# facebook/facebook360_dep

Hardware: AMD Instinct MI355X
Metric: depth Mpix/s per GPU (full pyramid, 16-cam 2048^2 rig); % HBM-read roofline (higher is better)
Workload: dtype f32+f64; 1 GPU; BASELINE config 3: 16-camera 2048x2048 synthetic rig, 8-frame sequence, full 10-level pyramid per frame, per-level temporal filter (+-2 frames); the same sequence for every --gpus N (block partition, 8 frame(s) on this rank); rig=cfg2, cameras=16, frames=8, temporal_filter=True, halo_transport=local, parallelism=frames x1

## Files before the change

### facebook360_dep_amd/csrc/derp_capi.hip

```cpp
#include <hip/hip_runtime.h>

#include <algorithm>
#include <cfloat>
#include <cmath>
#include <cstdarg>
#include <cstdio>
#include <cstdlib>
#include <cstring>
#include <map>
#include <memory>
#include <string>
#include <vector>

#include <rocprim/device/device_radix_sort.hpp>

#include "../../include/derp_hip.h"
#include "derp_host.h"
#include "derp_kernels.h"
#include "derp_mesh.h"
#include "derp_points.h"
#include "derp_render.h"
#include "derp_geometric.h"
#include "derp_sweep.h"

// ... 135 lines not shown
    coeffs[i] *= sum;
  }
}

int get_lanczos(derp_ctx* c, int ssize, int dsize, LanczosTab** out) {
  auto key = std::make_pair(ssize, dsize);
  auto it = c->lanczos.find(key);
  if (it != c->lanczos.end()) {
    *out = &it->second;
    return 0;
  }
  std::vector<int> ofs(dsize);
  std::vector<float> coef((size_t)dsize * 8);
  const double scale = (double)ssize / dsize;
  for (int d = 0; d < dsize; ++d) {
    float f = (float)((d + 0.5) * scale - 0.5);
    int s = (int)f;
    s -= (s > f);
    f -= s;
    ofs[d] = s;
    lanczos_coeffs(f, &coef[(size_t)d * 8]);
  }
  LanczosTab t;
  ALLOC(c, t.ofs, ofs.size() * sizeof(int));
  ALLOC(c, t.coef, coef.size() * sizeof(float));
  HIPCHK(c, hipMemcpyAsync(t.ofs.p, ofs.data(), ofs.size() * sizeof(int), hipMemcpyHostToDevice, c->stream));
  HIPCHK(c, hipMemcpyAsync(t.coef.p, coef.data(), coef.size() * sizeof(float), hipMemcpyHostToDevice, c->stream));
  HIPCHK(c, hipStreamSynchronize(c->stream));
  *out = &(c->lanczos[key] = std::move(t));
  return 0;
}

int get_area_tab(derp_ctx* c, int ssize, int dsize, AreaTabDev** out, bool forceTable = false) {
  auto key = std::make_pair(forceTable ? -ssize : ssize, dsize);
  auto it = c->areaTabs.find(key);
  if (it != c->areaTabs.end()) {
    *out = &it->second;
    return 0;
  }
  AreaTabDev t;
  const double scale = (double)ssize / dsize;
  const int iscale = (int)std::nearbyint(scale);
  std::vector<int> start(dsize + 1, 0), si;
  std::vector<float> alpha;
  if (!forceTable && iscale >= 1 && std::abs(scale - iscale) < 2.220446049250313e-16) {
    t.iscale = iscale;
// ... 96 lines not shown
  return locs;
}

int ensure_spiral(derp_ctx* c, int radius) {
  if (c->spiralRadius == radius) {
    return 0;
  }
  const std::vector<int2> s = make_spiral(radius * 2 + 1);
  ALLOC(c, c->spiral, s.size() * sizeof(int2));
  HIPCHK(c, hipMemcpy(c->spiral.p, s.data(), s.size() * sizeof(int2), hipMemcpyHostToDevice));
  c->spiralN = (int)s.size();
  c->spiralRadius = radius;
  return 0;
}

int upsample_lanczos_dev(derp_ctx* c, const float* in, int sw, int sh, float* out, int dw, int dh, int planes,
                         size_t inStride, size_t outStride) {
  if (sw == dw && sh == dh) {
    return fail(c, "upsample to identical size not supported");
  }
  LanczosTab *tx, *ty;
  TRY(get_lanczos(c, sw, dw, &tx));
  TRY(get_lanczos(c, sh, dh, &ty));
  const size_t tmpStride = (size_t)dw * sh;
  ALLOC(c, c->w.lanczosTmp, tmpStride * planes * sizeof(float));
  hipLaunchKernelGGL(k_lanczos_h, grid2d(dw, sh, planes, kBlk2d), kBlk2d, 0, c->stream, in, sw, sh, dw,
                     tx->ofs.as<int>(), tx->coef.as<float>(), c->w.lanczosTmp.as<float>(), inStride, tmpStride);
  KCHECK(c);
  hipLaunchKernelGGL(k_lanczos_v, grid2d(dw, dh, planes, kBlk2d), kBlk2d, 0, c->stream, c->w.lanczosTmp.as<float>(), sh,
                     dw, dh, ty->ofs.as<int>(), ty->coef.as<float>(), out, tmpStride, outStride);
  KCHECK(c);
  return 0;
}

int upsample_masked_dev(derp_ctx* c, const float* in, const uint8_t* mask, int sw, int sh, const uint8_t* maskUp,
                        const float* bgUp, float* out, int dw, int dh, int planes = 1) {
  const float scale = float(dw) / float(sw);
  const int radius = (int)(scale * scale + 1);
  TRY(ensure_spiral(c, radius));
  ALLOC(c, c->w.lanczosTmp, (size_t)dw * dh * planes * sizeof(float));
  hipLaunchKernelGGL(k_upsample_nearest_masked, grid2d(dw, dh, planes, kBlk2d), kBlk2d, 0, c->stream, in, mask, sw, sh,
                     maskUp, dw, dh, c->w.lanczosTmp.as<float>());
  KCHECK(c);
  hipLaunchKernelGGL(k_spiral_fill, grid2d(dw, dh, planes, kBlk2d), kBlk2d, 0, c->stream, c->w.lanczosTmp.as<float>(), bgUp,
                     maskUp, dw, dh, c->spiral.as<int2>(), c->spiralN, out);
  KCHECK(c);
// ... 136 lines not shown
  const int tiles = tilesX * tilesY;
  const size_t lds = kCostLdsPerSrc * (size_t)(c->S);
  const int run = std::min(std::max(c->bruteRun, 1), kNumDepths);
  hipLaunchKernelGGL(k_brute_costs, dim3(tiles, (kNumDepths + run - 1) / run, nd), dim3(kCostBlock), lds, c->stream, V,
                     c->w.bruteCost.as<float>(), c->w.bruteConf.as<float>(), tilesX, tiles, run);
  KCHECK(c);
  hipLaunchKernelGGL(k_brute_select, grid2d(V.W, V.H, nd, kBlk2d), kBlk2d, 0, c->stream, V, c->w.bruteCost.as<float>(),
                     c->w.bruteConf.as<float>());
  KCHECK(c);
  hipLaunchKernelGGL(k_brute_margin, grid2d(V.W, V.H, nd, kBlk2d), kBlk2d, 0, c->stream, V);
  KCHECK(c);
  return 0;
}

int run_random_proposals(derp_ctx* c, int dst0, int nd) {
  const int L = c->cur;
  if (c->opt.random_proposals <= 0 || L == c->numLevels - 1) {
    return 0;
  }
  Span sp(c, ST_RANDOM, L);
  c->randomRanThisLevel = true;
  LevelView V = make_view(c, ST_RANDOM, dst0, nd);
  if (V.H > 2 && V.W > 2) {
    hipLaunchKernelGGL(k_row_rank, dim3(V.H - 2, nd), dim3(256), 0, c->stream, V, c->w.rank.as<int>());
    KCHECK(c);
  }
  int tilesX;
  const int tiles = tiles_of(V.W, V.H, tilesX);
  const size_t lds = lds_for_waves(kCostLdsPerSrc * (size_t)(c->S), c->randomWaves, c->ldsPerCu, kCostLdsStatic);
  const CostGrid cg = cost_grid(c, tiles, tilesX, true);
  TRY(block_trace_attach(c, V, 0, cg.blocks, nd));
  const bool four = cost_four_waves(c);
  const auto kernel = cg.perBlock > 1 ? (four ? k_random_proposals_walk : k_random_proposals_walk_w3)
                                      : (four ? k_random_proposals : k_random_proposals_w3);
  hipLaunchKernelGGL(kernel, dim3(cg.blocks, nd), dim3(kCostBlock), lds, c->stream, V, c->w.rank.as<int>(), tilesX, cg.bands, cg.perBlock);
  KCHECK(c);
  return 0;
}

int run_ping_pong(derp_ctx* c, int dst0, int nd) {
  const int L = c->cur;
  if (L == c->numLevels - 1) {
    return 0;
  }
  Span sp(c, ST_PINGPONG, L);
  LevelView V = make_view(c, ST_PINGPONG, dst0, nd);
  const size_t n = (size_t)V.W * V.H;
// ... 135 lines not shown
  if (level < 0 || level >= c->numLevels) {
    return fail(c, "level %d out of range [0, %d)", level, c->numLevels);
  }
  if (c->LW[level] <= 0 || c->LH[level] <= 0) {
    return fail(c, "level %d was declared absent in derp_set_pyramid", level);
  }
  return 0;
}

int level_begin(derp_ctx* c, int level, bool buildAllTables) {
  TRY(check_level(c, level));
  if (c->S - 1 > kMaxSrc) {
    return fail(c, "too many source cameras (%d > %d)", c->S, kMaxSrc + 1);
  }
  c->cur = level;
  const int W = c->LW[level], H = c->LH[level];
  const size_t n = (size_t)W * H;
  if (W < 3 || H < 3) {
    return fail(c, "level %d is too small (%dx%d)", level, W, H);
  }
  TRY(compute_fov_and_masks(c, level));
  {
    Span sp(c, ST_VARIANCE, level);
    hipLaunchKernelGGL(k_variance, grid2d(W, H, c->S, kBlk2d), kBlk2d, 0, c->stream, c->frame().color[level].as<ushort4>(),
                       W, H, c->w.srcVar.as<float>());
    KCHECK(c);
  }
  {
    Span sp(c, ST_OWN_BIAS, level);
    hipLaunchKernelGGL(k_blur3_u16, blur_grid(W, H, c->S), kBlurBlk, 0, c->stream,
                       c->frame().color[level].as<ushort4>(), 0, c->w.ownBias.as<ushort4>(), 0, W, H, n, n);
    KCHECK(c);
  }
  HIPCHK(c, hipMemsetAsync(c->w.cost.p, 0, n * c->D * sizeof(float), c->stream));
  HIPCHK(c, hipMemsetAsync(c->w.confidence.p, 0, n * c->D * sizeof(float), c->stream));
  c->w.mismatchMaskHeld = level <= c->opt.mismatches_start_level && level != c->numLevels - 1;
  if (c->w.mismatchMaskHeld) {
    HIPCHK(c, hipMemsetAsync(c->w.mismatchMask.p, 0, n * c->D, c->stream));
  }
  if (level < c->numLevels - 1 && !c->frame().haveDisp[level + 1] && !buildAllTables) {
    return fail(c, "Missing disparity of level %d needed to start level %d", level + 1, level);
  }
  if (level < c->numLevels - 1 && c->frame().haveDisp[level + 1]) {
    Span sp(c, ST_UPSAMPLE, level);
    const int sw = c->LW[level + 1], sh = c->LH[level + 1];
    if (!c->opt.use_foreground_masks) {
      TRY(upsample_lanczos_dev(c, c->frame().disp[level + 1].as<float>(), sw, sh, c->w.disparity.as<float>(), W, H, c->D,
                               (size_t)sw * sh, n));
    } else {
      ALLOC(c, c->w.staging, (size_t)sw * sh * c->D);
      hipLaunchKernelGGL(k_fov_mask, grid2d(sw, sh, c->D, kBlk2d), kBlk2d, 0, c->stream, c->camsDst.as<Cam>(), sw, sh,
                         c->w.staging.as<uint8_t>());
      KCHECK(c);
      hipLaunchKernelGGL(k_and_masks, dim3(flat_grid((size_t)sw * sh), c->D), dim3(256), 0, c->stream,
// ... 791 lines not shown
```

### facebook360_dep_amd/csrc/derp_ctx.h

```cpp
#pragma once

namespace {

enum Stage {
  ST_FOV = 0,
  ST_VARIANCE,
  ST_OWN_BIAS,
  ST_UPSAMPLE,
  ST_PROJ_WARP,
  ST_REPROJECT,
  ST_PROJ_BIAS,
  ST_BRUTE,
  ST_RANDOM,
  ST_PINGPONG,
  ST_MISMATCH,
  ST_BILATERAL,
  ST_MEDIAN,
  ST_MASKFOV,
  ST_TEMPORAL,
  ST_LANES,
  ST_GC_PREPARE,
  ST_GC_SWEEP,
  ST_GC_CLEAN,
  ST_SWEEP_OVERLAPS,
  ST_SWEEP_EQUIRECT,
  ST_COUNT
};
const char* kStageNames[ST_COUNT] = {"fov_mask",  "variance",    "own_bias",         "upsample",  "proj_warp",
                                     "reproject", "proj_bias",   "brute_force",      "random_proposals",
                                     "ping_pong", "mismatches",  "bilateral",        "median",    "mask_fov",
                                     "temporal",  "lanes_wall", "gc_prepare",       "gc_sweep",  "gc_clean",
                                     "sweep_overlaps", "sweep_equirect"};
constexpr int kMaxLevels = 24;

struct TimedSpan {
  int stage, level;
  hipEvent_t a, b;
};

struct LanczosTab {
  DevBuf ofs, coef;
};

struct AreaTabDev {
  DevBuf start, si, alpha;
  int iscale = 0;
};

struct WorkSet {
  DevBuf srcVar, ownBias, maskAnd, disparity, cost, confidence, dispRes, costRes, changed, tmpF, rank, mismatchMask, pairCount;
  DevBuf tileSeen;
  DevBuf projColor, projBias;
  DevBuf projColorT;
  DevBuf bruteCost, bruteConf, lanczosTmp, staging, stagingB;
  bool mismatchMaskHeld = false;
  int colorTablesCleanLevel = -1;
};

struct FramePyramid {
  std::vector<DevBuf> color, fg, bg, disp;
  std::vector<char> haveBg, haveDisp;
};

struct WorkLane {
  hipStream_t stream = nullptr;
  hipEvent_t done = nullptr;
  WorkSet w;
};

struct SmrState; struct RephotoState; struct PointsState; struct MeshState; struct GcState; struct SweepState;

}

// ... 99 lines not shown
```

### facebook360_dep_amd/csrc/derp_debug_api.h

```cpp
#pragma once

namespace {
struct HostPairs {
  SsdPair* p;
  SsdPair get(int i) const {
    return p[i];
  }
  void set(int i, const SsdPair& v) {
    p[i] = v;
  }
};
int stage_index(const char* stage) {
  for (int i = 0; i < ST_COUNT; ++i) {
    if (strcmp(stage, kStageNames[i]) == 0) {
      return i;
    }
  }
  return -1;
}
}

int derp_debug_atan2_ypos(derp_ctx* c, const double* y, const double* x, double* out, size_t n) {
  if (!c || !y || !x || !out) {
    return fail(c, "bad arguments");
// ... 53 lines not shown
  }
  ALLOC(c, c->w.staging, 9 * n * sizeof(double));
  double* d = c->w.staging.as<double>();
  HIPCHK(c, hipMemcpyAsync(d, xyz, 3 * n * sizeof(double), hipMemcpyHostToDevice, c->stream));
  hipLaunchKernelGGL(k_debug_sees, dim3(flat_grid(n)), dim3(256), 0, c->stream, c->camsSrc.as<Cam>(), src, d, d + 3 * n, n);
  KCHECK(c);
  HIPCHK(c, hipMemcpyAsync(out, d + 3 * n, 6 * n * sizeof(double), hipMemcpyDeviceToHost, c->stream));
  HIPCHK(c, hipStreamSynchronize(c->stream));
  return 0;
}

int derp_debug_download(derp_ctx* c, int d, int s, int which, void* out) {
  TRY(need_current(c, false));
  const int L = c->cur;
  const int W = c->LW[L], H = c->LH[L];
  const size_t n = (size_t)W * H;
  HIPCHK(c, hipStreamSynchronize(c->stream));
  if (which == 4) {
    HIPCHK(c, hipMemcpy(out, c->w.srcVar.as<float>() + (size_t)s * n, n * sizeof(float), hipMemcpyDeviceToHost));
    return 0;
  }
  if (which == 5) {
    HIPCHK(c, hipMemcpy(out, c->fovMask.as<uint8_t>() + (size_t)d * n, n, hipMemcpyDeviceToHost));
    return 0;
  }
  if (d < 0 || d >= c->D || s < 0 || s >= c->S || s == c->dst2srcH[d]) {
    return fail(c, "bad (dst, src) pair");
  }
  const size_t tab = (size_t)d * (c->S - 1) + (s < c->dst2srcH[d] ? s : s - 1);
  if (which == 0) {
    const int PW = W + 2 * kPadW, PH = H + 2 * kPadW;
    std::vector<float2> tmp((size_t)PW * PH);
    HIPCHK(c, hipMemcpy(tmp.data(), c->projWarp.as<float2>() + tab * tmp.size(), tmp.size() * sizeof(float2),
                        hipMemcpyDeviceToHost));
    float2* o = reinterpret_cast<float2*>(out);
    for (int y = 0; y < H; ++y) {
      memcpy(o + (size_t)y * W, &tmp[(size_t)(y + kPadW) * PW + kPadW], (size_t)W * sizeof(float2));
    }
    return 0;
  }
  if (which == 2 || which == 3) {
    const int PW = W + 2 * kPadC, PH = H + 2 * kPadC;
    std::vector<ushort4> tmp((size_t)PW * PH);
    const ushort4* base = (which == 2 ? c->w.projColor.as<ushort4>() : c->w.projBias.as<ushort4>()) + tab * tmp.size();
    HIPCHK(c, hipMemcpy(tmp.data(), base, tmp.size() * sizeof(ushort4), hipMemcpyDeviceToHost));
    uint16_t* o = reinterpret_cast<uint16_t*>(out);
// ... 251 lines not shown
```

### facebook360_dep_amd/csrc/derp_kernels.h

```cpp
#pragma once
#include <hip/hip_runtime.h>
#include <math.h>
#include <stdint.h>

#include <type_traits>

#include "derp_camera.h"
#include "gcc_algos.h"

namespace derp {

#ifndef DERP_COST_MIN_WAVES
#define DERP_COST_MIN_WAVES 4
#endif
#ifndef DERP_RANDOM_MIN_WAVES
#define DERP_RANDOM_MIN_WAVES 4
#endif
#ifndef DERP_RANDOM_TILED
#define DERP_RANDOM_TILED 0
#endif
#ifndef DERP_MIX_HOT_ONLY
#define DERP_MIX_HOT_ONLY 0
#endif
#ifndef DERP_PHASE_TIMERS
// ... 853 lines not shown

__global__ void k_fov_mask(const Cam* __restrict__ cams, int W, int H, uint8_t* __restrict__ out) {
  const int d = blockIdx.z;
  const int x = blockIdx.x * blockDim.x + threadIdx.x, y = blockIdx.y * blockDim.y + threadIdx.y;
  if (x >= W || y >= H) {
    return;
  }
  const Cam& c = cams[d];
  const double px = (x + 0.5) / (double)W, py = (y + 0.5) / (double)H;
  out[(size_t)d * W * H + (size_t)y * W + x] =
      !outside_image_circle(c, px, py, c.principal[0], c.principal[1], c.focal[0], c.focal[1]);
}

__device__ __forceinline__ int reflect101(int p, int len) {
  if (len == 1) {
    return 0;
  }
  while (p < 0 || p >= len) {
    p = p < 0 ? -p : 2 * len - 2 - p;
  }
  return p;
}

__global__ void k_variance(const ushort4* __restrict__ color, int W, int H, float* __restrict__ var) {
  const int s = blockIdx.z;
  const int x = blockIdx.x * blockDim.x + threadIdx.x, y = blockIdx.y * blockDim.y + threadIdx.y;
  if (x >= W || y >= H) {
    return;
  }
  const ushort4* img = color + (size_t)s * W * H;
  const float scale = 1.0f / 65535.0f;
  double sum[3] = {0, 0, 0}, sumSq[3] = {0, 0, 0};
  const int xs[3] = {reflect101(x - 1, W), x, reflect101(x + 1, W)};
  for (int j = -1; j <= 1; ++j) {
    const int yy = reflect101(y + j, H);
    double rs[3], rq[3];
    {
      const ushort4 q0 = img[(size_t)yy * W + xs[0]], q1 = img[(size_t)yy * W + xs[1]], q2 = img[(size_t)yy * W + xs[2]];
      const float f0[3] = {q0.x * scale, q0.y * scale, q0.z * scale};
      const float f1[3] = {q1.x * scale, q1.y * scale, q1.z * scale};
      const float f2[3] = {q2.x * scale, q2.y * scale, q2.z * scale};
      for (int c = 0; c < 3; ++c) {
        rs[c] = (double)f0[c] + (double)f1[c] + (double)f2[c];
        rq[c] = (double)(f0[c] * f0[c]) + (double)(f1[c] * f1[c]) + (double)(f2[c] * f2[c]);
      }
    }
    for (int c = 0; c < 3; ++c) {
      sum[c] += rs[c];
      sumSq[c] += rq[c];
    }
  }
  const double k = 1. / 9;
  float v[3];
  for (int c = 0; c < 3; ++c) {
    const float mean = (float)(sum[c] * k);
    const float meanSq = (float)(sumSq[c] * k);
    v[c] = meanSq - mean * mean;
  }
  const float t = v[0] * 0.3333f + v[1] * 0.3334f;
  var[(size_t)s * W * H + (size_t)y * W + x] = t * 1.0f + v[2] * 0.3333f;
}

constexpr int kBlurRows = 8;
__device__ __forceinline__ ushort4 blur3_texel(const ushort4* __restrict__ img, int IW, int padIn, int W, int H, int x,
                                               int y) {
  unsigned s0 = 0, s1 = 0, s2 = 0;
  for (int j = -1; j <= 1; ++j) {
    const int yy = reflect101(y + j, H) + padIn;
    for (int i = -1; i <= 1; ++i) {
      const int xx = reflect101(x + i, W) + padIn;
      const ushort4 q = img[(size_t)yy * IW + xx];
      s0 += q.x;
      s1 += q.y;
      s2 += q.z;
    }
  }
  return make_ushort4((unsigned short)((s0 + 4) / 9), (unsigned short)((s1 + 4) / 9), (unsigned short)((s2 + 4) / 9), 0);
}
__global__ void k_blur3_u16(const ushort4* __restrict__ in, int padIn, ushort4* __restrict__ out, int padOut, int W,
                            int H, size_t planeIn, size_t planeOut) {
  const int p = blockIdx.z;
  const int ox = blockIdx.x * blockDim.x + threadIdx.x;
  const int oy0 = (blockIdx.y * blockDim.y + threadIdx.y) * kBlurRows;
  const int OW = W + 2 * padOut, OH = H + 2 * padOut;
  if (ox >= OW || oy0 >= OH) {
    return;
  }
  const ushort4* img = in + (size_t)p * planeIn;
  ushort4* dst = out + (size_t)p * planeOut;
  const int IW = W + 2 * padIn;
  const int x = ox - padOut, y0 = oy0 - padOut;
  if (x >= 1 && x <= W - 2 && y0 >= 1 && y0 + kBlurRows - 1 <= H - 2) {
    auto hsum = [&](int y, unsigned (&h)[3]) {
      const ushort4* r = img + (size_t)(y + padIn) * IW + (x + padIn);
      const ushort4 a = r[-1], b = r[0], c = r[1];
      h[0] = (unsigned)a.x + b.x + c.x;
      h[1] = (unsigned)a.y + b.y + c.y;
      h[2] = (unsigned)a.z + b.z + c.z;
    };
    unsigned hp[3], hc[3], hn[3];
    hsum(y0 - 1, hp);
    hsum(y0, hc);
#pragma unroll
    for (int r = 0; r < kBlurRows; ++r) {
      hsum(y0 + r + 1, hn);
      dst[(size_t)(oy0 + r) * OW + ox] =
          make_ushort4((unsigned short)((hp[0] + hc[0] + hn[0] + 4) / 9), (unsigned short)((hp[1] + hc[1] + hn[1] + 4) / 9),
                       (unsigned short)((hp[2] + hc[2] + hn[2] + 4) / 9), 0);
#pragma unroll
      for (int c = 0; c < 3; ++c) {
        hp[c] = hc[c];
        hc[c] = hn[c];
      }
    }
    return;
  }
  const int xc = min(max(x, 0), W - 1);
  for (int r = 0; r < kBlurRows && oy0 + r < OH; ++r) {
    const int yc = min(max(y0 + r, 0), H - 1);
    dst[(size_t)(oy0 + r) * OW + ox] = blur3_texel(img, IW, padIn, W, H, xc, yc);
  }
}

__global__ void k_proj_warp(LevelView V, float2* __restrict__ projWarp) {
  const int s = blockIdx.z;
  const int ox = blockIdx.x * blockDim.x + threadIdx.x, oy = blockIdx.y * blockDim.y + threadIdx.y;
  const int OW = V.W + 2 * kPadW, OH = V.H + 2 * kPadW;
  if (ox >= OW || oy >= OH) {
    return;
  }
  const int x = min(max(ox - kPadW, 0), V.W - 1), y = min(max(oy - kPadW, 0), V.H - 1);
  const Cam& cs = V.camsSrc[s];
  const double W = V.W, H = V.H;
  const double sprx = cs.principal[0] * W, spry = cs.principal[1] * H, sfx = cs.focal[0] * W, sfy = cs.focal[1] * H;
  const double px = x + 0.5, py = y + 0.5;
  const bool outside = outside_image_circle(cs, px, py, sprx, spry, sfx, sfy);
  D3 rig = {0, 0, 0};
  if (!outside) {
    const D3 dir = rig_direction(cs, px, py, sprx, spry, sfx, sfy);
    rig = {cs.pos[0] + dir.x * 1e4, cs.pos[1] + dir.y * 1e4, cs.pos[2] + dir.z * 1e4};
  }
  const size_t plane = (size_t)OW * OH;
  const float nan = __builtin_nanf("");
// ... 518 lines not shown
  const int own = V.dst2src[d];
  const size_t n = (size_t)V.W * V.H, idx = (size_t)y * V.W + x;
  if (!V.srcFg[(size_t)own * n + idx]) {
    V.disparity[(size_t)d * n + idx] = V.bgDisp[(size_t)d * n + idx];
    return;
  }
  const int yy = min(max(y, 1), V.H - 2), xx = min(max(x, 1), V.W - 2);
  const size_t src = (size_t)yy * V.W + xx;
  V.disparity[(size_t)d * n + idx] = V.disparity[(size_t)d * n + src];
  V.cost[(size_t)d * n + idx] = V.cost[(size_t)d * n + src];
  V.confidence[(size_t)d * n + idx] = V.confidence[(size_t)d * n + src];
}

__device__ __forceinline__ bool random_gate(const LevelView& V, int d, int own, size_t idx) {
  const size_t n = (size_t)V.W * V.H;
  if (!V.fovMask[(size_t)d * n + idx] || !V.srcFg[(size_t)own * n + idx]) {
    return false;
  }
  const float varHighDev = 0.1f * V.varHighThresh;
  const float thresh = fmaxf(varHighDev, V.varNoiseFloor);
  return !(V.srcVar[(size_t)own * n + idx] < thresh);
}

__global__ void __launch_bounds__(256) k_row_rank(LevelView V, int* __restrict__ rank) {
  __shared__ int partial[256];
  const int d = V.dst0 + blockIdx.y, y = blockIdx.x + 1;
  const int own = V.dst2src[d];
  const size_t n = (size_t)V.W * V.H;
  const int inner = V.W - 2;
  const int per = (inner + 255) / 256;
  const int x0 = 1 + threadIdx.x * per, x1 = min(x0 + per, V.W - 1);
  int cnt = 0;
  for (int x = x0; x < x1; ++x) {
    cnt += random_gate(V, d, own, (size_t)y * V.W + x);
  }
  partial[threadIdx.x] = cnt;
  __syncthreads();
  for (int off = 1; off < 256; off <<= 1) {
    const int v = ((int)threadIdx.x >= off) ? partial[threadIdx.x - off] : 0;
    __syncthreads();
    partial[threadIdx.x] += v;
    __syncthreads();
  }
  const int run = partial[threadIdx.x] - cnt;
  uint32_t state = minstd_jump(minstd_seed(y * V.level), (uint64_t)V.randomProposals * (uint64_t)run);
  const uint32_t aP = minstd_jump(1u, (uint64_t)V.randomProposals);
  for (int x = x0; x < x1; ++x) {
    rank[(size_t)d * n + (size_t)y * V.W + x] = (int)state;
    if (random_gate(V, d, own, (size_t)y * V.W + x)) {
      state = minstd_mulmod(state, aP);
    }
  }
}

__device__ __forceinline__ void random_proposals_tile(const LevelView& V, const int* __restrict__ rank, int dl, int x, int y, bool go,
                                                      const PatchWin* win, LdsPairs& pairs) {
  const int d = V.dst0 + dl;
  const int own = V.dst2src[d];
  const size_t n = (size_t)V.W * V.H;
  const unsigned idx = (unsigned)y * (unsigned)V.W + (unsigned)x;
  float* disp = V.disparity + (size_t)d * n;
  unsigned nCost = 0, nPair = 0, nSlots = 0, nSlotsFirst = 0;
  PhaseTimers tm;
  const unsigned tk0 = phase_clock();
  if (go) {
    PixCtx px;
    load_pixctx<false>(V, d, own, x, y, win, px);
    const unsigned cull = behind_sources(V, d, idx);
    float currDisp = at32(disp, idx);
    float currCost = 0.f, costThresh = 0.f, amplitude = 0.f;
    const int spare = V.S - 1;
    const float maxDisp = 1.0f / V.minDepthM;
    uint32_t state = (uint32_t)at32(rank + (size_t)d * n, idx);
// ... 712 lines not shown
  if (mask[idx]) {
    const float4 centre = bilateral_texel<GUIDE_U16>(guideV, idx, result);
    const float denom = 2.0f * (sigma * sigma);
    const double rcpDenom = 1.0 / (double)denom;
    float sumWeight = 0.f, weightedAvg = 0.f;
    for (int v = -radius; v <= radius; ++v) {
      const size_t row = (size_t)min(max(y + v, 0), H - 1) * W;
      for (int u = -radius; u <= radius; ++u) {
        const size_t j = row + min(max(x + u, 0), W - 1);
        if (!mask[j]) {
          continue;
        }
        bilateral_tap(centre, bilateral_texel<GUIDE_U16>(guideV, j, image[j]), weight0, weight1, weight2, rcpDenom,
                      expTab, sumWeight, weightedAvg);
      }
    }
    if (sumWeight != 0.0f) {
      result = weightedAvg / sumWeight;
    }
  }
  out[idx] = result;
}

__device__ __forceinline__ void cswap(float& a, float& b) {
  const float lo = fminf(a, b), hi = fmaxf(a, b);
  a = lo;
  b = hi;
}

__global__ void k_masked_median(const float* __restrict__ image, const float* __restrict__ background,
                                const uint8_t* __restrict__ mask, int W, int H, int radius, float* __restrict__ out,
                                size_t planeStride, const uint8_t* __restrict__ fovForNan) {
  const int p = blockIdx.z;
  const int x = blockIdx.x * blockDim.x + threadIdx.x, y = blockIdx.y * blockDim.y + threadIdx.y;
  if (x >= W || y >= H) {
    return;
  }
  const size_t idx = (size_t)y * W + x;
  const float* img = image + (size_t)p * planeStride;
  const uint8_t* m = mask + (size_t)p * planeStride;
  float result = 0.0f;
  if (!m[idx]) {
    if (background) {
      result = background[(size_t)p * planeStride + idx];
    }
  } else if (radius == 1) {
    const float inf = __builtin_inff();
    float v[9];
    int cnt = 0;
#pragma unroll
    for (int j = 0; j < 3; ++j) {
#pragma unroll
      for (int i = 0; i < 3; ++i) {
        const int yy = y + j - 1, xx = x + i - 1;
        float t = inf;
        if (yy >= 0 && yy < H && xx >= 0 && xx < W) {
          const size_t q = (size_t)yy * W + xx;
          const float val = img[q];
          if (m[q] && !isnan(val) && val != 0) {
            t = val;
            ++cnt;
          }
        }
        v[j * 3 + i] = t;
      }
    }
    cswap(v[0], v[1]); cswap(v[3], v[4]); cswap(v[6], v[7]);
    cswap(v[1], v[2]); cswap(v[4], v[5]); cswap(v[7], v[8]);
    cswap(v[0], v[1]); cswap(v[3], v[4]); cswap(v[6], v[7]);
    cswap(v[0], v[3]); cswap(v[3], v[6]); cswap(v[0], v[3]);
    cswap(v[1], v[4]); cswap(v[4], v[7]); cswap(v[1], v[4]);
    cswap(v[2], v[5]); cswap(v[5], v[8]); cswap(v[2], v[5]);
    cswap(v[1], v[3]); cswap(v[5], v[7]); cswap(v[2], v[6]);
    cswap(v[4], v[6]); cswap(v[2], v[4]); cswap(v[2], v[3]);
    cswap(v[5], v[6]);
    if (cnt > 0) {
      const int h = cnt / 2;
      float lo = v[0], hi = v[0];
#pragma unroll
      for (int k = 0; k < 9; ++k) {
        lo = (k == h - 1) ? v[k] : lo;
        hi = (k == h) ? v[k] : hi;
      }
      result = (cnt & 1) ? hi : (float)(((double)(lo + hi)) / 2.0);
    }
  } else {
    float vals[25];
// ... 79 lines not shown
    v += sv * a[j];
  }
  tmp[(size_t)p * tmpStride + (size_t)y * DW + dx] = v;
}
__global__ void k_lanczos_v(const float* __restrict__ tmp, int SH, int DW, int DH, const int* __restrict__ yofs,
                            const float* __restrict__ beta, float* __restrict__ out, size_t tmpStride,
                            size_t outStride) {
  const int p = blockIdx.z;
  const int x = blockIdx.x * blockDim.x + threadIdx.x, dy = blockIdx.y * blockDim.y + threadIdx.y;
  if (x >= DW || dy >= DH) {
    return;
  }
  const float* T = tmp + (size_t)p * tmpStride;
  const float* b = beta + (size_t)dy * 8;
  const int sy = yofs[dy] - 3;
  float r[8];
#pragma unroll
  for (int k = 0; k < 8; ++k) {
    const int syk = min(max(sy + k, 0), SH - 1);
    r[k] = T[(size_t)syk * DW + x];
  }
  out[(size_t)p * outStride + (size_t)dy * DW + x] =
      r[0] * b[0] + r[1] * b[1] + r[2] * b[2] + r[3] * b[3] + r[4] * b[4] + r[5] * b[5] + r[6] * b[6] + r[7] * b[7];
}

__global__ void k_upsample_nearest_masked(const float* __restrict__ in, const uint8_t* __restrict__ mask, int SW,
                                          int SH, const uint8_t* __restrict__ maskUp, int DW, int DH,
                                          float* __restrict__ out) {
  const int x = blockIdx.x * blockDim.x + threadIdx.x, y = blockIdx.y * blockDim.y + threadIdx.y;
  if (x >= DW || y >= DH) {
    return;
  }
  {
    const size_t ps = (size_t)blockIdx.z * SW * SH, pd = (size_t)blockIdx.z * DW * DH;
    in += ps;
    mask += ps;
    maskUp += pd;
    out += pd;
  }
  const double ifx = (double)SW / DW, ify = (double)SH / DH;
  const int sx = min((int)floor(x * ifx), SW - 1), sy = min((int)floor(y * ify), SH - 1);
  float v = in[(size_t)sy * SW + sx];
  if (!mask[(size_t)sy * SW + sx] || !maskUp[(size_t)y * DW + x]) {
    v = __builtin_nanf("");
  }
  out[(size_t)y * DW + x] = v;
// ... 944 lines not shown
```

### facebook360_dep_amd/derp.py

```python
import ctypes as C
import os

import numpy as np

_HERE = os.path.dirname(os.path.abspath(__file__))
LIB_PATH = os.environ.get("DERP_LIB") or os.path.join(_HERE, "libderp_hip.so")
CAM_TYPES = {"FTHETA": 0, "RECTILINEAR": 1, "EQUISOLID": 2, "ORTHOGRAPHIC": 3}

STAGES = ["fov_mask", "variance", "own_bias", "upsample", "proj_warp", "reproject", "proj_bias", "brute_force",
          "random_proposals", "ping_pong", "mismatches", "bilateral", "median", "mask_fov", "temporal"]


class SeqOptions(C.Structure):
    _fields_ = [
        ("time_radius", C.c_int32), ("sigma", C.c_float), ("weight_b", C.c_float), ("weight_g", C.c_float),
        ("weight_r", C.c_float), ("space_radius", C.c_int32), ("use_foreground_masks", C.c_int32),
        ("partition", C.c_int32), ("do_temporal_filter", C.c_int32), ("resident_frames", C.c_int32),
    ]


class SeqTransfer(C.Structure):
    _fields_ = [("frame", C.c_int32), ("from_rank", C.c_int32), ("to_rank", C.c_int32)]


# ... 377 lines not shown
        assert b is None or b.shape == a.shape
        out = np.zeros_like(a)
        self._ck(lib().derp_debug_fp64(self.h, self.FP64_OPS[op], _p(a), _p(b), _p(out), C.c_size_t(a.size)))
        return out

    def debug_expf(self, x, nonpos=False):
        x = np.ascontiguousarray(x, np.float32)
        out = np.zeros_like(x)
        self._ck(lib().derp_debug_expf(self.h, int(bool(nonpos)), _p(x), _p(out), C.c_size_t(x.size)))
        return out

    def debug_sees(self, src, xyz):
        xyz = np.ascontiguousarray(xyz, np.float64).reshape(-1, 3)
        out = np.zeros((len(xyz), 2, 3))
        self._ck(lib().derp_debug_sees(self.h, src, _p(xyz), C.c_size_t(len(xyz)), _p(out)))
        return out[:, :, 0].T != 0, np.ascontiguousarray(out[:, :, 1:].transpose(1, 0, 2))

    def debug(self, d, s, which):
        h, w = self._shape(self._cur)
        spec = {"warp": (0, (h, w, 2), np.float32), "color": (2, (h, w, 3), np.uint16),
                "bias": (3, (h, w, 3), np.uint16), "variance": (4, (h, w), np.float32),
                "fov": (5, (h, w), np.uint8),
                "color_padded": (6, (h + 4, w + 4, 4), np.uint16), "bias_padded": (7, (h + 4, w + 4, 4), np.uint16),
                "tile_seen": (8, ((h + 31) // 32, (w + 31) // 32), np.uint8)}[which]
        out = np.zeros(spec[1], dtype=spec[2])
        self._ck(lib().derp_debug_download(self.h, d, s, spec[0], _p(out)))
        return out

    def mismatch_mask(self, d):
        out = np.zeros(self._shape(self._cur), dtype=np.uint8)
        self._ck(lib().derp_download_mismatch_mask(self.h, d, _p(out)))
        return out

    def layer_disparities(self, fg, bg):
        fg = np.ascontiguousarray(fg, dtype=np.float32)
        bg = np.ascontiguousarray(bg, dtype=np.float32)
        out = np.zeros(fg.shape, dtype=np.uint8)
        self._ck(lib().derp_layer_disparities(self.h, _p(fg), _p(bg), C.c_size_t(fg.size), _p(out)))
        return out

    def ssim(self, x, y, blur_radius=1, alpha=1.0, beta=1.0, gamma=1.0):
        x = np.ascontiguousarray(x, dtype=np.float32)
        y = np.ascontiguousarray(y, dtype=np.float32)
        h, w = x.shape[:2]
        out = np.zeros((h, w, 3), dtype=np.float32)
        self._ck(lib().derp_ssim(self.h, _p(x), _p(y), w, h, blur_radius, C.c_float(alpha), C.c_float(beta),
                                 C.c_float(gamma), _p(out)))
# ... 753 lines not shown
```

Baseline: 519.6 Mpix/s.

## Fuse variance/bias, single-pass Lanczos, ballot-based row rank, LDS median taps

Several independent changes. Variance and own-bias blur are merged into one kernel that streams 8 rows per thread, so the colour image is read once instead of twice. Lanczos upsampling gets a single-pass tiled kernel that keeps horizontal results in LDS, skipping the temporary buffer. k_row_rank uses wave ballots and a precomputed table of minstd powers instead of a serial per-thread scan, and the radius-1 masked median loads its taps into LDS. These mainly target memory traffic and serial work in small stages, at the cost of more LDS use and more kernel complexity; the fused variance kernel also drops the old interior fast path of the blur.

```diff
diff --git a/facebook360_dep_amd/csrc/derp_capi.hip b/facebook360_dep_amd/csrc/derp_capi.hip
--- a/facebook360_dep_amd/csrc/derp_capi.hip
+++ b/facebook360_dep_amd/csrc/derp_capi.hip
@@ -181,6 +181,12 @@
     lanczos_coeffs(f, &coef[(size_t)d * 8]);
   }
   LanczosTab t;
+  for (int d0 = 0; d0 < dsize; d0 += kLanczosH) {
+    const int d1 = std::min(d0 + kLanczosH, dsize) - 1;
+    const int lo = std::min(std::max(ofs[d0] - 3, 0), ssize - 1), hi = std::min(std::max(ofs[d1] + 4, 0), ssize - 1);
+    t.tileSpan = std::max(t.tileSpan, hi - lo + 1);
+    t.monotone = t.monotone && std::is_sorted(ofs.begin() + d0, ofs.begin() + d1 + 1);
+  }
   ALLOC(c, t.ofs, ofs.size() * sizeof(int));
   ALLOC(c, t.coef, coef.size() * sizeof(float));
   HIPCHK(c, hipMemcpyAsync(t.ofs.p, ofs.data(), ofs.size() * sizeof(int), hipMemcpyHostToDevice, c->stream));
@@ -323,6 +329,13 @@
   LanczosTab *tx, *ty;
   TRY(get_lanczos(c, sw, dw, &tx));
   TRY(get_lanczos(c, sh, dh, &ty));
+  if (ty->monotone && ty->tileSpan <= kLanczosRows) {
+    hipLaunchKernelGGL(k_lanczos, dim3((dw + kLanczosW - 1) / kLanczosW, (dh + kLanczosH - 1) / kLanczosH, planes),
+                       dim3(kLanczosW, 4), 0, c->stream, in, sw, sh, dw, dh, tx->ofs.as<int>(), tx->coef.as<float>(),
+                       ty->ofs.as<int>(), ty->coef.as<float>(), out, inStride, outStride);
+    KCHECK(c);
+    return 0;
+  }
   const size_t tmpStride = (size_t)dw * sh;
   ALLOC(c, c->w.lanczosTmp, tmpStride * planes * sizeof(float));
   hipLaunchKernelGGL(k_lanczos_h, grid2d(dw, sh, planes, kBlk2d), kBlk2d, 0, c->stream, in, sw, sh, dw,
@@ -505,7 +518,18 @@
   c->randomRanThisLevel = true;
   LevelView V = make_view(c, ST_RANDOM, dst0, nd);
   if (V.H > 2 && V.W > 2) {
-    hipLaunchKernelGGL(k_row_rank, dim3(V.H - 2, nd), dim3(256), 0, c->stream, V, c->w.rank.as<int>());
+    WorkSet& w = c->w;
+    if (w.rankPowersP != V.randomProposals || w.rankPowersN < V.W) {
+      const int count = *std::max_element(c->LW.begin(), c->LW.end());
+      ALLOC(c, w.rankPowers, (size_t)count * sizeof(uint32_t));
+      hipLaunchKernelGGL(k_minstd_powers, dim3(blocks_of(count, 256)), dim3(256), 0, c->stream, V.randomProposals, count,
+                         w.rankPowers.as<uint32_t>());
+      KCHECK(c);
+      w.rankPowersP = V.randomProposals;
+      w.rankPowersN = count;
+    }
+    hipLaunchKernelGGL(k_row_rank, dim3(V.H - 2, nd), dim3(256), 0, c->stream, V, w.rankPowers.as<uint32_t>(),
+                       w.rank.as<int>());
     KCHECK(c);
   }
   int tilesX;
@@ -687,14 +711,8 @@
   TRY(compute_fov_and_masks(c, level));
   {
     Span sp(c, ST_VARIANCE, level);
-    hipLaunchKernelGGL(k_variance, grid2d(W, H, c->S, kBlk2d), kBlk2d, 0, c->stream, c->frame().color[level].as<ushort4>(),
-                       W, H, c->w.srcVar.as<float>());
-    KCHECK(c);
-  }
-  {
-    Span sp(c, ST_OWN_BIAS, level);
-    hipLaunchKernelGGL(k_blur3_u16, blur_grid(W, H, c->S), kBlurBlk, 0, c->stream,
-                       c->frame().color[level].as<ushort4>(), 0, c->w.ownBias.as<ushort4>(), 0, W, H, n, n);
+    hipLaunchKernelGGL(k_variance_bias, blur_grid(W, H, c->S), kBlurBlk, 0, c->stream, c->frame().color[level].as<ushort4>(),
+                       W, H, c->w.srcVar.as<float>(), c->w.ownBias.as<ushort4>());
     KCHECK(c);
   }
   HIPCHK(c, hipMemsetAsync(c->w.cost.p, 0, n * c->D * sizeof(float), c->stream));
diff --git a/facebook360_dep_amd/csrc/derp_ctx.h b/facebook360_dep_amd/csrc/derp_ctx.h
--- a/facebook360_dep_amd/csrc/derp_ctx.h
+++ b/facebook360_dep_amd/csrc/derp_ctx.h
@@ -40,6 +40,8 @@
 
 struct LanczosTab {
   DevBuf ofs, coef;
+  int tileSpan = 0;
+  bool monotone = true;
 };
 
 struct AreaTabDev {
@@ -49,6 +51,8 @@
 
 struct WorkSet {
   DevBuf srcVar, ownBias, maskAnd, disparity, cost, confidence, dispRes, costRes, changed, tmpF, rank, mismatchMask, pairCount;
+  DevBuf rankPowers;
+  int rankPowersP = -1, rankPowersN = 0;
   DevBuf tileSeen;
   DevBuf projColor, projBias;
   DevBuf projColorT;
diff --git a/facebook360_dep_amd/csrc/derp_debug_api.h b/facebook360_dep_amd/csrc/derp_debug_api.h
--- a/facebook360_dep_amd/csrc/derp_debug_api.h
+++ b/facebook360_dep_amd/csrc/derp_debug_api.h
@@ -99,6 +99,27 @@
   }
   if (which == 5) {
     HIPCHK(c, hipMemcpy(out, c->fovMask.as<uint8_t>() + (size_t)d * n, n, hipMemcpyDeviceToHost));
+    return 0;
+  }
+  if (which == 9) {
+    if (s < 0 || s >= c->S) {
+      return fail(c, "bad source index");
+    }
+    std::vector<ushort4> tmp(n);
+    HIPCHK(c, hipMemcpy(tmp.data(), c->w.ownBias.as<ushort4>() + (size_t)s * n, n * sizeof(ushort4), hipMemcpyDeviceToHost));
+    uint16_t* o = reinterpret_cast<uint16_t*>(out);
+    for (size_t i = 0; i < n; ++i) {
+      o[i * 3 + 0] = tmp[i].x;
+      o[i * 3 + 1] = tmp[i].y;
+      o[i * 3 + 2] = tmp[i].z;
+    }
+    return 0;
+  }
+  if (which == 10) {
+    if (d < 0 || d >= c->D) {
+      return fail(c, "bad destination index");
+    }
+    HIPCHK(c, hipMemcpy(out, c->w.rank.as<int>() + (size_t)d * n, n * sizeof(int), hipMemcpyDeviceToHost));
     return 0;
   }
   if (d < 0 || d >= c->D || s < 0 || s >= c->S || s == c->dst2srcH[d]) {
diff --git a/facebook360_dep_amd/csrc/derp_kernels.h b/facebook360_dep_amd/csrc/derp_kernels.h
--- a/facebook360_dep_amd/csrc/derp_kernels.h
+++ b/facebook360_dep_amd/csrc/derp_kernels.h
@@ -899,103 +899,71 @@
   return p;
 }
 
-__global__ void k_variance(const ushort4* __restrict__ color, int W, int H, float* __restrict__ var) {
+constexpr int kBlurRows = 8;
+struct BoxRow {
+  unsigned h[3];
+  double rs[3], rq[3];
+};
+__global__ void __launch_bounds__(256) k_variance_bias(const ushort4* __restrict__ color, int W, int H,
+                                                       float* __restrict__ var, ushort4* __restrict__ bias) {
   const int s = blockIdx.z;
-  const int x = blockIdx.x * blockDim.x + threadIdx.x, y = blockIdx.y * blockDim.y + threadIdx.y;
-  if (x >= W || y >= H) {
-    return;
-  }
-  const ushort4* img = color + (size_t)s * W * H;
+  const int x = blockIdx.x * blockDim.x + threadIdx.x;
+  const int y0 = (blockIdx.y * blockDim.y + threadIdx.y) * kBlurRows;
+  if (x >= W || y0 >= H) {
+    return;
+  }
+  const size_t n = (size_t)W * H;
+  const ushort4* img = color + (size_t)s * n;
+  const int xl = reflect101(x - 1, W), xr = reflect101(x + 1, W);
   const float scale = 1.0f / 65535.0f;
-  double sum[3] = {0, 0, 0}, sumSq[3] = {0, 0, 0};
-  const int xs[3] = {reflect101(x - 1, W), x, reflect101(x + 1, W)};
-  for (int j = -1; j <= 1; ++j) {
-    const int yy = reflect101(y + j, H);
-    double rs[3], rq[3];
-    {
-      const ushort4 q0 = img[(size_t)yy * W + xs[0]], q1 = img[(size_t)yy * W + xs[1]], q2 = img[(size_t)yy * W + xs[2]];
-      const float f0[3] = {q0.x * scale, q0.y * scale, q0.z * scale};
-      const float f1[3] = {q1.x * scale, q1.y * scale, q1.z * scale};
-      const float f2[3] = {q2.x * scale, q2.y * scale, q2.z * scale};
-      for (int c = 0; c < 3; ++c) {
-        rs[c] = (double)f0[c] + (double)f1[c] + (double)f2[c];
-        rq[c] = (double)(f0[c] * f0[c]) + (double)(f1[c] * f1[c]) + (double)(f2[c] * f2[c]);
-      }
-    }
+  auto row_sums = [&](int y, BoxRow& r) {
+    const ushort4* line = img + (size_t)reflect101(y, H) * W;
+    const ushort4 q0 = line[xl], q1 = line[x], q2 = line[xr];
+    r.h[0] = (unsigned)q0.x + q1.x + q2.x;
+    r.h[1] = (unsigned)q0.y + q1.y + q2.y;
+    r.h[2] = (unsigned)q0.z + q1.z + q2.z;
+    const float f0[3] = {q0.x * scale, q0.y * scale, q0.z * scale};
+    const float f1[3] = {q1.x * scale, q1.y * scale, q1.z * scale};
+    const float f2[3] = {q2.x * scale, q2.y * scale, q2.z * scale};
+#pragma unroll
     for (int c = 0; c < 3; ++c) {
-      sum[c] += rs[c];
-      sumSq[c] += rq[c];
-    }
-  }
+      r.rs[c] = (double)f0[c] + (double)f1[c] + (double)f2[c];
+      r.rq[c] = (double)(f0[c] * f0[c]) + (double)(f1[c] * f1[c]) + (double)(f2[c] * f2[c]);
+    }
+  };
+  BoxRow rp, rc, rn;
+  row_sums(y0 - 1, rp);
+  row_sums(y0, rc);
   const double k = 1. / 9;
-  float v[3];
-  for (int c = 0; c < 3; ++c) {
-    const float mean = (float)(sum[c] * k);
-    const float meanSq = (float)(sumSq[c] * k);
-    v[c] = meanSq - mean * mean;
-  }
-  const float t = v[0] * 0.3333f + v[1] * 0.3334f;
-  var[(size_t)s * W * H + (size_t)y * W + x] = t * 1.0f + v[2] * 0.3333f;
-}
-
-constexpr int kBlurRows = 8;
-__device__ __forceinline__ ushort4 blur3_texel(const ushort4* __restrict__ img, int IW, int padIn, int W, int H, int x,
-                                               int y) {
-  unsigned s0 = 0, s1 = 0, s2 = 0;
-  for (int j = -1; j <= 1; ++j) {
-    const int yy = reflect101(y + j, H) + padIn;
-    for (int i = -1; i <= 1; ++i) {
-      const int xx = reflect101(x + i, W) + padIn;
-      const ushort4 q = img[(size_t)yy * IW + xx];
-      s0 += q.x;
-      s1 += q.y;
-      s2 += q.z;
-    }
-  }
-  return make_ushort4((unsigned short)((s0 + 4) / 9), (unsigned short)((s1 + 4) / 9), (unsigned short)((s2 + 4) / 9), 0);
-}
-__global__ void k_blur3_u16(const ushort4* __restrict__ in, int padIn, ushort4* __restrict__ out, int padOut, int W,
-                            int H, size_t planeIn, size_t planeOut) {
-  const int p = blockIdx.z;
-  const int ox = blockIdx.x * blockDim.x + threadIdx.x;
-  const int oy0 = (blockIdx.y * blockDim.y + threadIdx.y) * kBlurRows;
-  const int OW = W + 2 * padOut, OH = H + 2 * padOut;
-  if (ox >= OW || oy0 >= OH) {
-    return;
-  }
-  const ushort4* img = in + (size_t)p * planeIn;
-  ushort4* dst = out + (size_t)p * planeOut;
-  const int IW = W + 2 * padIn;
-  const int x = ox - padOut, y0 = oy0 - padOut;
-  if (x >= 1 && x <= W - 2 && y0 >= 1 && y0 + kBlurRows - 1 <= H - 2) {
-    auto hsum = [&](int y, unsigned (&h)[3]) {
-      const ushort4* r = img + (size_t)(y + padIn) * IW + (x + padIn);
-      const ushort4 a = r[-1], b = r[0], c = r[1];
-      h[0] = (unsigned)a.x + b.x + c.x;
-      h[1] = (unsigned)a.y + b.y + c.y;
-      h[2] = (unsigned)a.z + b.z + c.z;
-    };
-    unsigned hp[3], hc[3], hn[3];
-    hsum(y0 - 1, hp);
-    hsum(y0, hc);
-#pragma unroll
-    for (int r = 0; r < kBlurRows; ++r) {
-      hsum(y0 + r + 1, hn);
-      dst[(size_t)(oy0 + r) * OW + ox] =
-          make_ushort4((unsigned short)((hp[0] + hc[0] + hn[0] + 4) / 9), (unsigned short)((hp[1] + hc[1] + hn[1] + 4) / 9),
-                       (unsigned short)((hp[2] + hc[2] + hn[2] + 4) / 9), 0);
-#pragma unroll
-      for (int c = 0; c < 3; ++c) {
-        hp[c] = hc[c];
-        hc[c] = hn[c];
-      }
-    }
-    return;
-  }
-  const int xc = min(max(x, 0), W - 1);
-  for (int r = 0; r < kBlurRows && oy0 + r < OH; ++r) {
-    const int yc = min(max(y0 + r, 0), H - 1);
-    dst[(size_t)(oy0 + r) * OW + ox] = blur3_texel(img, IW, padIn, W, H, xc, yc);
+#pragma unroll
+  for (int r = 0; r < kBlurRows; ++r) {
+    const int y = y0 + r;
+    if (y >= H) {
+      break;
+    }
+    row_sums(y + 1, rn);
+    float v[3];
+#pragma unroll
+    for (int c = 0; c < 3; ++c) {
+      double sum = 0, sumSq = 0;
+      sum += rp.rs[c];
+      sumSq += rp.rq[c];
+      sum += rc.rs[c];
+      sumSq += rc.rq[c];
+      sum += rn.rs[c];
+      sumSq += rn.rq[c];
+      const float mean = (float)(sum * k);
+      const float meanSq = (float)(sumSq * k);
+      v[c] = meanSq - mean * mean;
+    }
+    const float t = v[0] * 0.3333f + v[1] * 0.3334f;
+    const size_t idx = (size_t)y * W + x;
+    var[(size_t)s * n + idx] = t * 1.0f + v[2] * 0.3333f;
+    bias[(size_t)s * n + idx] = make_ushort4((unsigned short)((rp.h[0] + rc.h[0] + rn.h[0] + 4) / 9),
+                                             (unsigned short)((rp.h[1] + rc.h[1] + rn.h[1] + 4) / 9),
+                                             (unsigned short)((rp.h[2] + rc.h[2] + rn.h[2] + 4) / 9), 0);
+    rp = rc;
+    rc = rn;
   }
 }
 
@@ -1560,33 +1528,39 @@
   return !(V.srcVar[(size_t)own * n + idx] < thresh);
 }
 
-__global__ void __launch_bounds__(256) k_row_rank(LevelView V, int* __restrict__ rank) {
-  __shared__ int partial[256];
+__global__ void k_minstd_powers(int proposals, int count, uint32_t* __restrict__ powers) {
+  const int k = blockIdx.x * blockDim.x + threadIdx.x;
+  if (k < count) {
+    powers[k] = minstd_jump(1u, (uint64_t)proposals * (uint64_t)k);
+  }
+}
+
+__global__ void __launch_bounds__(256) k_row_rank(LevelView V, const uint32_t* __restrict__ powers, int* __restrict__ rank) {
+  __shared__ int waveCount[2][4];
   const int d = V.dst0 + blockIdx.y, y = blockIdx.x + 1;
   const int own = V.dst2src[d];
   const size_t n = (size_t)V.W * V.H;
-  const int inner = V.W - 2;
-  const int per = (inner + 255) / 256;
-  const int x0 = 1 + threadIdx.x * per, x1 = min(x0 + per, V.W - 1);
-  int cnt = 0;
-  for (int x = x0; x < x1; ++x) {
-    cnt += random_gate(V, d, own, (size_t)y * V.W + x);
-  }
-  partial[threadIdx.x] = cnt;
-  __syncthreads();
-  for (int off = 1; off < 256; off <<= 1) {
-    const int v = ((int)threadIdx.x >= off) ? partial[threadIdx.x - off] : 0;
+  const int lane = threadIdx.x & 63, wave = threadIdx.x >> 6;
+  const uint32_t seed = minstd_seed(y * V.level);
+  int before = 0;
+  for (int xb = 1, step = 0; xb < V.W - 1; xb += 256, ++step) {
+    const int x = xb + (int)threadIdx.x;
+    const size_t idx = (size_t)y * V.W + x;
+    const bool go = x < V.W - 1 && random_gate(V, d, own, idx);
+    const unsigned long long ballot = __ballot(go);
+    if (lane == 0) {
+      waveCount[step & 1][wave] = __popcll(ballot);
+    }
     __syncthreads();
-    partial[threadIdx.x] += v;
-    __syncthreads();
-  }
-  const int run = partial[threadIdx.x] - cnt;
-  uint32_t state = minstd_jump(minstd_seed(y * V.level), (uint64_t)V.randomProposals * (uint64_t)run);
-  const uint32_t aP = minstd_jump(1u, (uint64_t)V.randomProposals);
-  for (int x = x0; x < x1; ++x) {
-    rank[(size_t)d * n + (size_t)y * V.W + x] = (int)state;
-    if (random_gate(V, d, own, (size_t)y * V.W + x)) {
-      state = minstd_mulmod(state, aP);
+    int k = before + __popcll(ballot & ((1ull << lane) - 1ull));
+#pragma unroll
+    for (int w = 0; w < 4; ++w) {
+      const int t = waveCount[step & 1][w];
+      k += w < wave ? t : 0;
+      before += t;
+    }
+    if (go) {
+      rank[(size_t)d * n + idx] = (int)minstd_mulmod(seed, powers[k]);
     }
   }
 }
@@ -2345,6 +2319,7 @@
   out[idx] = result;
 }
 
+constexpr int kMedianBlkW = 32, kMedianBlkH = 8;
 __device__ __forceinline__ void cswap(float& a, float& b) {
   const float lo = fminf(a, b), hi = fmaxf(a, b);
   a = lo;
@@ -2354,14 +2329,33 @@
 __global__ void k_masked_median(const float* __restrict__ image, const float* __restrict__ background,
                                 const uint8_t* __restrict__ mask, int W, int H, int radius, float* __restrict__ out,
                                 size_t planeStride, const uint8_t* __restrict__ fovForNan) {
+  __shared__ float taps[kMedianBlkH + 2][kMedianBlkW + 2];
   const int p = blockIdx.z;
   const int x = blockIdx.x * blockDim.x + threadIdx.x, y = blockIdx.y * blockDim.y + threadIdx.y;
-  if (x >= W || y >= H) {
-    return;
-  }
-  const size_t idx = (size_t)y * W + x;
   const float* img = image + (size_t)p * planeStride;
   const uint8_t* m = mask + (size_t)p * planeStride;
+  if (radius == 1) {
+    const int tw = (int)blockDim.x + 2, th = (int)blockDim.y + 2;
+    const int x0 = (int)(blockIdx.x * blockDim.x) - 1, y0 = (int)(blockIdx.y * blockDim.y) - 1;
+    for (int i = threadIdx.y * blockDim.x + threadIdx.x; i < tw * th; i += blockDim.x * blockDim.y) {
+      const int ty = i / tw, tx = i - ty * tw;
+      const int yy = y0 + ty, xx = x0 + tx;
+      float t = __builtin_nanf("");
+      if (yy >= 0 && yy < H && xx >= 0 && xx < W) {
+        const size_t q = (size_t)yy * W + xx;
+        const float val = img[q];
+        if (m[q] && val != 0) {
+          t = val;
+        }
+      }
+      taps[ty][tx] = t;
+    }
+    __syncthreads();
+  }
+  if (x >= W || y >= H) {
+    return;
+  }
+  const size_t idx = (size_t)y * W + x;
   float result = 0.0f;
   if (!m[idx]) {
     if (background) {
@@ -2375,17 +2369,10 @@
     for (int j = 0; j < 3; ++j) {
 #pragma unroll
       for (int i = 0; i < 3; ++i) {
-        const int yy = y + j - 1, xx = x + i - 1;
-        float t = inf;
-        if (yy >= 0 && yy < H && xx >= 0 && xx < W) {
-          const size_t q = (size_t)yy * W + xx;
-          const float val = img[q];
-          if (m[q] && !isnan(val) && val != 0) {
-            t = val;
-            ++cnt;
-          }
-        }
-        v[j * 3 + i] = t;
+        const float val = taps[threadIdx.y + j][threadIdx.x + i];
+        const bool valid = !isnan(val);
+        cnt += valid;
+        v[j * 3 + i] = valid ? val : inf;
       }
     }
     cswap(v[0], v[1]); cswap(v[3], v[4]); cswap(v[6], v[7]);
@@ -2511,6 +2498,51 @@
   }
   out[(size_t)p * outStride + (size_t)dy * DW + x] =
       r[0] * b[0] + r[1] * b[1] + r[2] * b[2] + r[3] * b[3] + r[4] * b[4] + r[5] * b[5] + r[6] * b[6] + r[7] * b[7];
+}
+constexpr int kLanczosW = 64, kLanczosH = 32, kLanczosRows = 40;
+__global__ void __launch_bounds__(256) k_lanczos(const float* __restrict__ in, int SW, int SH, int DW, int DH,
+                                                 const int* __restrict__ xofs, const float* __restrict__ alpha,
+                                                 const int* __restrict__ yofs, const float* __restrict__ beta,
+                                                 float* __restrict__ out, size_t inStride, size_t outStride) {
+  __shared__ float rows[kLanczosRows][kLanczosW];
+  const int p = blockIdx.z;
+  const int dx = blockIdx.x * kLanczosW + threadIdx.x;
+  const int dy0 = blockIdx.y * kLanczosH, dy1 = min(dy0 + kLanczosH, DH) - 1;
+  const int rowLo = min(max(yofs[dy0] - 3, 0), SH - 1), rowHi = min(max(yofs[dy1] + 4, 0), SH - 1);
+  if (dx < DW) {
+    const float* a = alpha + (size_t)dx * 8;
+    const int sx = xofs[dx] - 3;
+    for (int r = threadIdx.y; r <= rowHi - rowLo && r < kLanczosRows; r += blockDim.y) {
+      const float* S = in + (size_t)p * inStride + (size_t)(rowLo + r) * SW;
+      float v = 0;
+#pragma unroll
+      for (int j = 0; j < 8; ++j) {
+        const int sxj = min(max(sx + j, 0), SW - 1);
+        float sv = S[sxj];
+        if (sv != sv) {
+          sv = 1e-4f;
+        }
+        v += sv * a[j];
+      }
+      rows[r][threadIdx.x] = v;
+    }
+  }
+  __syncthreads();
+  if (dx >= DW) {
+    return;
+  }
+  for (int dy = dy0 + threadIdx.y; dy <= dy1; dy += blockDim.y) {
+    const float* b = beta + (size_t)dy * 8;
+    const int sy = yofs[dy] - 3;
+    float r[8];
+#pragma unroll
+    for (int k = 0; k < 8; ++k) {
+      const int syk = min(max(sy + k, 0), SH - 1);
+      r[k] = rows[min(syk - rowLo, kLanczosRows - 1)][threadIdx.x];
+    }
+    out[(size_t)p * outStride + (size_t)dy * DW + dx] =
+        r[0] * b[0] + r[1] * b[1] + r[2] * b[2] + r[3] * b[3] + r[4] * b[4] + r[5] * b[5] + r[6] * b[6] + r[7] * b[7];
+  }
 }
 
 __global__ void k_upsample_nearest_masked(const float* __restrict__ in, const uint8_t* __restrict__ mask, int SW,
diff --git a/facebook360_dep_amd/derp.py b/facebook360_dep_amd/derp.py
--- a/facebook360_dep_amd/derp.py
+++ b/facebook360_dep_amd/derp.py
@@ -423,7 +423,8 @@
                 "bias": (3, (h, w, 3), np.uint16), "variance": (4, (h, w), np.float32),
                 "fov": (5, (h, w), np.uint8),
                 "color_padded": (6, (h + 4, w + 4, 4), np.uint16), "bias_padded": (7, (h + 4, w + 4, 4), np.uint16),
-                "tile_seen": (8, ((h + 31) // 32, (w + 31) // 32), np.uint8)}[which]
+                "tile_seen": (8, ((h + 31) // 32, (w + 31) // 32), np.uint8),
+                "own_bias": (9, (h, w, 3), np.uint16), "rank": (10, (h, w), np.uint32)}[which]
         out = np.zeros(spec[1], dtype=spec[2])
         self._ck(lib().derp_debug_download(self.h, d, s, spec[0], _p(out)))
         return out
```

Result: faster. 527.7 Mpix/s (median of 6 runs) (+1.6%).
